# dask-contrib/dask-sql

Hardware: NVIDIA H100
Metric: rows/s on Q3-shaped filter->join->groupby (higher is better)
Workload: dtype f64

## Files before the change

dask-sql_b200/_lib.py:

```python
import ctypes as C
import os

HERE = os.path.dirname(os.path.abspath(__file__))
LIB_PATH = os.environ.get("B200SQL_LIB") or os.path.join(HERE, "libb200sql.so")

I64, F64, U8 = 0, 1, 2
U32 = 3
COL_SENTINEL = 1
MAX_COLS, MAX_TERMS, MAX_AGGS, MAX_KEYS, MAX_GATHER, MAX_PROG = 16, 8, 8, 4, 8, 64
TILE = 4096
EQ, NE, LT, LE, GT, GE, IS_NULL, IS_NOT_NULL, IS_TRUE = range(9)
AGG_SUM, AGG_SUMF, AGG_MIN, AGG_MAX, AGG_COUNT, AGG_AND, AGG_OR, AGG_XOR = range(8)
JOIN_INNER, JOIN_LEFT, JOIN_SEMI, JOIN_ANTI = range(4)
EMPTY_KEY = -(1 << 63)

OP_LOAD, OP_CONST_I, OP_CONST_F, OP_CONST_NULL, OP_I2F, OP_F2I = 0, 1, 2, 3, 4, 5
OP_ADD_I, OP_SUB_I, OP_MUL_I, OP_DIV_I, OP_NEG_I, OP_ABS_I, OP_MOD_I = 10, 11, 12, 13, 14, 15, 16
OP_ADD_F, OP_SUB_F, OP_MUL_F, OP_DIV_F, OP_NEG_F, OP_ABS_F, OP_SQRT_F = 20, 21, 22, 23, 24, 25, 26
OP_EQ_I, OP_EQ_F = 30, 40
OP_AND, OP_OR, OP_NOT, OP_ISNULL_I, OP_ISNULL_F, OP_CASE, OP_FILLNA, OP_ORD2F = 50, 51, 52, 53, 54, 55, 56, 57
OP_DATEPART, OP_ADDMONTHS = 60, 61
(DP_DAYS, DP_YEAR, DP_QUARTER, DP_MONTH, DP_DAY, DP_DOY, DP_DOW, DP_ISOWEEK, DP_HOUR, DP_MINUTE, DP_SECOND,
 DP_MILLISECOND, DP_MICROSECOND) = range(13)

# ... 48 lines not shown
                ("range", C.c_int64), ("table_keys", C.c_void_p), ("table_slots", C.c_void_p),
                ("cap", C.c_int64), ("dir", C.c_void_p)]


MAX_PEERS, PEER_MAX_ARRAYS = 16, 2 * MAX_AGGS + 1
PEER_SUM_F64, PEER_SUM_I64, PEER_MIN_I64, PEER_MAX_I64, PEER_AND_I64, PEER_OR_I64, PEER_XOR_I64 = range(7)
PEER_PRESENT_ROWS, PEER_PRESENT_INDICATOR, PEER_PRESENT_BITMAP = 1, 2, 3


class PeerMerge(C.Structure):
    _fields_ = [("world", C.c_int32), ("rank", C.c_int32), ("narrays", C.c_int32), ("presence_kind", C.c_int32),
                ("presence_array", C.c_int32), ("ops", C.c_int32 * PEER_MAX_ARRAYS),
                ("array_off", C.c_int64 * PEER_MAX_ARRAYS), ("bitmap_off", C.c_int64), ("signal_off", C.c_int64),
                ("peer_base", C.c_void_p * MAX_PEERS), ("out", C.c_void_p * PEER_MAX_ARRAYS),
                ("out_present", C.c_void_p), ("lo", C.c_int64), ("count", C.c_int64), ("local_ready", C.c_void_p),
                ("epoch", C.c_uint64)]


assert C.sizeof(Col) == 24 and C.sizeof(Term) == 32 and C.sizeof(Scan) == 656
assert C.sizeof(AggState) == 152 and C.sizeof(Instr) == 24 and C.sizeof(Prog) == 1544
assert C.sizeof(JoinTable) == 152 and C.sizeof(StarLookup) == 64 and C.sizeof(PeerMerge) == 544


def agg_identity(op):
    return {AGG_MIN: (1 << 63) - 1, AGG_MAX: -(1 << 63), AGG_AND: -1}.get(op, 0)


class B200SqlError(RuntimeError):
    pass


def _load():
    if not os.path.exists(LIB_PATH):
        raise ImportError(
            f"{LIB_PATH} is missing: the execution layer has no CPU fallback. Build it with "
            "`python __graft_entry__.py build` (nvcc -gencode arch=compute_90a,code=sm_90a).")
    return C.CDLL(LIB_PATH)


_lib = _load()
_lib.b2_last_error.restype = C.c_char_p
_lib.b2_num_tiles.restype = C.c_int64
_lib.b2_num_tiles.argtypes = [C.c_int64]
_lib.b2_stats_ws_bytes.restype = C.c_int64
_lib.b2_scan_agg_ws_bytes.restype = C.c_int64
_lib.b2_join_onepass_ws_bytes.restype = C.c_int64
_lib.b2_join_onepass_ws_bytes.argtypes = [C.c_int64]
_lib.b2_range_partition_ws_bytes.restype = C.c_int64
_lib.b2_range_partition_ws_bytes.argtypes = [C.c_int32]
_lib.b2_f64_to_ordered.restype = C.c_int64
_lib.b2_f64_to_ordered.argtypes = [C.c_double]
_lib.b2_ordered_to_f64.restype = C.c_double
_lib.b2_ordered_to_f64.argtypes = [C.c_int64]

_P = C.c_void_p
_SIGS = {
    "b2_version": [],
    "b2_device_info": [C.c_int32, C.POINTER(C.c_int32), C.POINTER(C.c_int64), C.POINTER(C.c_int32),
                       C.POINTER(C.c_int32), C.POINTER(C.c_int64)],
    "b2_d2h": [_P, _P, C.c_int64, _P],
    "b2_sync": [_P],
    "b2_memset": [_P, C.c_int32, C.c_int64, _P],
    "b2_col_stats": [C.POINTER(Col), C.c_int64, _P, _P, _P],
    "b2_expr_eval": [C.POINTER(Prog), C.POINTER(Col), C.c_int32, C.c_int64, _P, _P, _P],
    "b2_scan_agg": [C.POINTER(Scan), C.POINTER(Agg), C.c_int32, _P, _P, C.c_int32, _P, _P],
    "b2_select_count": [C.POINTER(Scan), _P, _P],
    "b2_select_write": [C.POINTER(Scan), _P, _P, C.c_int32, C.POINTER(C.c_int32), C.POINTER(_P),
                        C.POINTER(_P), _P],
    "b2_gather": [C.POINTER(Col), _P, C.c_int64, _P, _P, _P],
    "b2_groupby_dense": [C.POINTER(Scan), C.c_int32, C.c_int64, C.c_int64, C.POINTER(Agg), C.c_int32,
                         C.POINTER(AggState), _P],
    "b2_groupby_dense_grouped": [C.POINTER(Scan), C.c_int32, C.c_int64, C.c_int64, C.POINTER(Agg), C.c_int32,
                                 C.POINTER(AggState), _P],
    "b2_hot_slots": [C.POINTER(Col), C.c_int64, C.c_int64, C.c_int64, _P, _P],
    "b2_groupby_dense_hot": [C.POINTER(Scan), C.c_int32, C.c_int64, C.c_int64, C.POINTER(Agg), C.c_int32,
                             C.POINTER(AggState), _P, _P],
    "b2_groupby_dense_ordered": [C.POINTER(Scan), C.c_int32, C.c_int64, C.c_int64, C.POINTER(Agg), C.c_int32,
                                 C.POINTER(AggState), _P, _P],
    "b2_groupby_hash1": [C.POINTER(Scan), C.c_int32, _P, C.c_int64, C.POINTER(Agg), C.c_int32,
                         C.POINTER(AggState), _P, _P],
    "b2_groupby_hashk": [C.POINTER(Scan), C.POINTER(C.c_int32), C.c_int32, _P, _P, _P, C.c_int64,
                         C.POINTER(Agg), C.c_int32, C.POINTER(AggState), _P, _P],
    "b2_join_build": [C.POINTER(Col), C.c_int32, C.c_int64, _P, _P, C.c_int64, _P],
    "b2_join_build_dense": [C.POINTER(Col), C.c_int64, C.c_int64, C.c_int64, _P, _P, _P],
    "b2_join_count": [C.POINTER(Scan), C.POINTER(C.c_int32), C.POINTER(JoinTable), C.c_int32, _P, _P],
    "b2_join_write": [C.POINTER(Scan), C.POINTER(C.c_int32), C.POINTER(JoinTable), C.c_int32, _P, _P, _P,
                      _P, _P],
    "b2_join_write_gather": [C.POINTER(Scan), C.POINTER(C.c_int32), C.POINTER(JoinTable), C.c_int32, _P, _P, _P,
                             _P, C.c_int32, C.POINTER(C.c_int32), C.POINTER(_P), C.POINTER(_P), C.c_int32,
                             C.POINTER(Col), C.POINTER(_P), C.POINTER(_P), _P],
    "b2_join_key_layout": [C.POINTER(Col), C.c_int64, C.c_int64, C.c_int64, C.POINTER(Col), C.c_int32, C.c_int64,
                           _P, _P, _P, _P],
    "b2_join_write_gather_keyed": [C.POINTER(Scan), C.POINTER(C.c_int32), C.POINTER(JoinTable), C.c_int32, _P, _P,
                                   _P, _P, C.c_int32, C.POINTER(C.c_int32), C.POINTER(_P), C.POINTER(_P),
                                   C.c_int32, C.POINTER(Col), C.POINTER(C.c_int64), C.POINTER(_P), C.POINTER(_P),
                                   _P],
    "b2_join_onepass": [C.POINTER(Scan), C.POINTER(C.c_int32), C.POINTER(JoinTable), C.c_int32, C.c_int32, _P, C.c_int32,
                        C.POINTER(C.c_int32), C.POINTER(_P), C.POINTER(_P), C.c_int32, C.POINTER(Col),
                        C.POINTER(C.c_int64), C.POINTER(_P), C.POINTER(_P), _P],
    "b2_join_agg": [C.POINTER(Scan), C.c_int32, C.POINTER(JoinTable), C.c_int32, C.POINTER(Col), C.POINTER(C.c_int64),
                    C.POINTER(JoinAgg), C.c_int32, _P, _P, C.c_int32, _P, _P],
    "b2_range_partition_hist": [C.POINTER(Scan), C.c_int32, C.c_int64, C.c_int64, C.c_int32, C.c_int32, _P, _P],
    "b2_range_partition_scan": [C.c_int32, _P, _P],
    "b2_range_partition_scatter": [C.POINTER(Scan), C.c_int32, C.c_int64, C.c_int64, C.c_int32, C.c_int32, C.c_int32,
                                   C.POINTER(C.c_int32), _P, C.POINTER(_P), _P, _P],
    "b2_range_partition": [C.POINTER(Scan), C.c_int32, C.c_int64, C.c_int64, C.c_int32, C.c_int32, C.c_int32,
                           C.POINTER(C.c_int32), _P, C.POINTER(_P), _P, _P],
    "b2_iota": [_P, C.c_int64, _P],
    "b2_bitwise_combine": [_P, _P, C.c_int64, C.c_int32, _P],
    "b2_peer_merge": [C.POINTER(PeerMerge), _P],
    "b2_sort_by": [C.POINTER(Col), C.c_int64, C.c_int32, C.c_int32, _P, _P, _P],
    "b2_dense_slots": [C.POINTER(Col), C.c_int64, C.c_int64, C.c_int32, _P, _P],
    "b2_star_build_dense": [C.POINTER(Col), _P, C.c_int64, _P, C.c_int64, C.c_int64, _P, _P, _P],
    "b2_star_build_mark": [C.POINTER(Scan), C.c_int32, C.c_int64, C.c_int64, _P, _P, _P],
    "b2_star_build_rank": [_P, C.c_int64, _P],
    "b2_star_build_fill": [C.POINTER(Scan), C.c_int32, C.c_int32, C.c_int64, C.c_int64, C.c_int64, C.c_int32, _P,
                           _P, _P],
    "b2_star_build_fill_packed": [C.POINTER(Scan), C.c_int32, C.c_int32, C.c_int64, C.c_int64, C.c_int64,
                                  C.c_int32, _P, _P, C.c_int32, _P],
    "b2_star_build_hash": [C.POINTER(Col), _P, C.c_int64, _P, _P, _P, C.c_int64, _P, _P],
    "b2_star_agg": [C.POINTER(Scan), C.c_int32, C.POINTER(StarLookup), C.POINTER(Agg), C.c_int32,
                    C.POINTER(AggState), _P],
}

EXPORTS = sorted(list(_SIGS) + ["b2_last_error", "b2_num_tiles", "b2_stats_ws_bytes", "b2_scan_agg_ws_bytes",
                                "b2_sort_ws_bytes", "b2_join_onepass_ws_bytes", "b2_range_partition_ws_bytes",
                                "b2_f64_to_ordered", "b2_ordered_to_f64"])


call_times = {} if os.environ.get("B200SQL_CALL_TIMES") == "1" else None


def _wrap(name):
    fn = getattr(_lib, name)
    fn.restype = C.c_int32
    fn.argtypes = _SIGS[name]

    if call_times is not None:
        import time

        def call(*args):
            t0 = time.perf_counter()
            rc = fn(*args)
            rec = call_times.setdefault(name, [0, 0.0])
            rec[0] += 1
            rec[1] += time.perf_counter() - t0
            if rc != 0:
                raise B200SqlError(f"{name} failed ({rc}): {_lib.b2_last_error().decode()}")
            return rc

        call.__name__ = name
        return call

    def call(*args):
        rc = fn(*args)
        if rc != 0:
            raise B200SqlError(f"{name} failed ({rc}): {_lib.b2_last_error().decode()}")
        return rc

    call.__name__ = name
    return call


version = getattr(_lib, "b2_version")
version.restype = C.c_int32
device_info = _wrap("b2_device_info")
d2h = _wrap("b2_d2h")
sync = _wrap("b2_sync")
memset = _wrap("b2_memset")
col_stats = _wrap("b2_col_stats")
expr_eval = _wrap("b2_expr_eval")
scan_agg = _wrap("b2_scan_agg")
select_count = _wrap("b2_select_count")
select_write = _wrap("b2_select_write")
gather = _wrap("b2_gather")
groupby_dense = _wrap("b2_groupby_dense")
groupby_dense_ordered = _wrap("b2_groupby_dense_ordered")
groupby_dense_grouped = _wrap("b2_groupby_dense_grouped")
groupby_dense_hot = _wrap("b2_groupby_dense_hot")
hot_slots = _wrap("b2_hot_slots")
groupby_hash1 = _wrap("b2_groupby_hash1")
groupby_hashk = _wrap("b2_groupby_hashk")
join_build = _wrap("b2_join_build")
join_build_dense = _wrap("b2_join_build_dense")
join_count = _wrap("b2_join_count")
join_write = _wrap("b2_join_write")
join_write_gather = _wrap("b2_join_write_gather")
join_write_gather_keyed = _wrap("b2_join_write_gather_keyed")
join_key_layout = _wrap("b2_join_key_layout")
join_onepass = _wrap("b2_join_onepass")
join_onepass_ws_bytes = _lib.b2_join_onepass_ws_bytes
join_agg = _wrap("b2_join_agg")
range_partition = _wrap("b2_range_partition")
range_partition_hist = _wrap("b2_range_partition_hist")
range_partition_scan = _wrap("b2_range_partition_scan")
range_partition_scatter = _wrap("b2_range_partition_scatter")
range_partition_ws_bytes = _lib.b2_range_partition_ws_bytes
iota = _wrap("b2_iota")
bitwise_combine = _wrap("b2_bitwise_combine")
peer_merge = _wrap("b2_peer_merge")
sort_by = _wrap("b2_sort_by")
_lib.b2_sort_ws_bytes.restype = C.c_int64
_lib.b2_sort_ws_bytes.argtypes = [C.c_int64]
sort_ws_bytes = _lib.b2_sort_ws_bytes
dense_slots = _wrap("b2_dense_slots")
star_build_dense = _wrap("b2_star_build_dense")
star_build_mark = _wrap("b2_star_build_mark")
star_build_rank = _wrap("b2_star_build_rank")
star_build_fill = _wrap("b2_star_build_fill")
star_build_fill_packed = _wrap("b2_star_build_fill_packed")
star_build_hash = _wrap("b2_star_build_hash")
star_agg = _wrap("b2_star_agg")
num_tiles = _lib.b2_num_tiles
stats_ws_bytes = _lib.b2_stats_ws_bytes
scan_agg_ws_bytes = _lib.b2_scan_agg_ws_bytes
f64_to_ordered = _lib.b2_f64_to_ordered
ordered_to_f64 = _lib.b2_ordered_to_f64


def has_symbol(name):
    try:
        getattr(_lib, name)
        return True
    except AttributeError:
        return False
```

dask-sql_b200/csrc/groupby.cuh:

```cuda
#pragma once
#include "common.cuh"
#include "pipeline.cuh"
#include "warpagg.cuh"

#define B2_GB_R 8
#define B2_GB_ROWS_PER_BLOCK (B2_BLOCK * B2_GB_R)
#define B2_MAX_PROBE 1024

template <int R, class LD>
__device__ __forceinline__ void b2_dense_slots_of(const b2_scan_t& s, const LD& ld, int key_col, int64_t kmin,
                                                  int64_t nslots, int64_t (&slot)[R]) {
  const b2_col_t& kc = s.cols[key_col];
  bool full;
  const uint32_t bits = b2_eval_terms<R>(s, ld, full);
  int64_t key[R];
  ld.template load<R>(key_col, bits, full, key);
  uint32_t kvalid = bits;
  if (kc.valid) kvalid = b2_valid_bits<R>(kc.valid, ld.row0, bits);
#pragma unroll
  for (int j = 0; j < R; ++j) {
    slot[j] = -1;
    if ((bits >> j) & 1) {
      if (!((kvalid >> j) & 1)) slot[j] = nslots - 1;
      else {
// ... 210 lines not shown
b2_star_build_dense_kernel(const __grid_constant__ b2_col_t pk, const int32_t* __restrict__ sel, int64_t n_sel,
                           const int32_t* __restrict__ slot_of_row, int64_t kmin, int64_t range,
                           int32_t* __restrict__ lookup, int32_t* __restrict__ flags) {
  for (int64_t i = (int64_t)blockIdx.x * B2_BLOCK + threadIdx.x; i < n_sel; i += (int64_t)gridDim.x * B2_BLOCK) {
    const int64_t r = sel ? sel[i] : i;
    const int64_t raw = b2_load_raw(pk, r);
    if (b2_is_null(pk, r, raw)) continue;
    const uint64_t d = (uint64_t)raw - (uint64_t)kmin;
    if (d >= (uint64_t)range) continue;
    const int32_t old = atomicExch(lookup + d, slot_of_row[i]);
    if (old != -1) flags[0] = 1;
  }
}

__device__ __forceinline__ uint32_t b2_slot_word(uint32_t pos, int slot_bits) {
  return slot_bits == 16 ? pos >> 2 : __umulhi(pos, 0x55555556u);
}

template <bool FILL>
__global__ void __launch_bounds__(B2_BLOCK)
b2_star_build_scan_kernel(const __grid_constant__ b2_scan_t s, int pk_col, int grp_col, int64_t pk_min,
                          int64_t pk_range, int64_t grp_min, int32_t null_slot, uint64_t* __restrict__ dir,
                          void* __restrict__ slots, int slot_bits, int32_t* __restrict__ flags) {
  const int tile_off = (threadIdx.x >> 5) * (32 * B2_GB_R) + (threadIdx.x & 31);
  const b2_col_t& pc = s.cols[pk_col];
  const b2_col_t& gc = s.cols[grp_col];
  for (int64_t base = (int64_t)blockIdx.x * B2_GB_ROWS_PER_BLOCK; base < s.n;
       base += (int64_t)gridDim.x * B2_GB_ROWS_PER_BLOCK) {
    const b2_gld ld{&s, base + tile_off};
    bool full;
    const uint32_t bits = b2_eval_terms<B2_GB_R>(s, ld, full);
    int64_t pk[B2_GB_R];
    ld.template load<B2_GB_R>(pk_col, bits, full, pk);
    uint32_t live = bits;
    if (pc.valid) live &= b2_valid_bits<B2_GB_R>(pc.valid, ld.row0, bits);
#pragma unroll
    for (int j = 0; j < B2_GB_R; ++j) {
      const uint64_t d = (uint64_t)pk[j] - (uint64_t)pk_min;
      if (!(((live >> j) & 1) && d < (uint64_t)pk_range)) live &= ~(1u << j);
    }
    if (!FILL) {
#pragma unroll
      for (int j = 0; j < B2_GB_R; ++j) {
        if (!((live >> j) & 1)) continue;
        const uint64_t d = (uint64_t)pk[j] - (uint64_t)pk_min;
        const uint32_t b = 1u << (d & 31);
        if (atomicOr(reinterpret_cast<uint32_t*>(dir + (d >> 5)), b) & b) flags[0] = 1;
      }
    } else {
      int64_t grp[B2_GB_R];
      ld.template load<B2_GB_R>(grp_col, live, false, grp);
      uint32_t gnull = 0;
      if (gc.valid) gnull = live & ~b2_valid_bits<B2_GB_R>(gc.valid, ld.row0, live);
#pragma unroll
      for (int j = 0; j < B2_GB_R; ++j) {
        if (!((live >> j) & 1)) continue;
        const uint64_t d = (uint64_t)pk[j] - (uint64_t)pk_min;
        const uint64_t w = dir[d >> 5];
        const uint32_t pos = (uint32_t)(w >> 32) + __popc((uint32_t)w & ((1u << (d & 31)) - 1));
        const int32_t v = (gnull >> j) & 1 ? null_slot : (int32_t)(grp[j] - grp_min);
        if (slot_bits == 32) {
          static_cast<int32_t*>(slots)[pos] = v;
        } else {
          const uint32_t q = b2_slot_word(pos, slot_bits);
          const uint32_t sh = (pos - q * (64 / slot_bits)) * slot_bits;
          unsigned long long* p = reinterpret_cast<unsigned long long*>(slots) + q;
          const unsigned long long m = ((1ull << slot_bits) - 1) << sh;
          const unsigned long long e = ((unsigned long long)(uint32_t)v << sh) & m;
          unsigned long long old = 0, seen;
          while ((seen = atomicCAS(p, old, (old & ~m) | e)) != old) old = seen;
        }
      }
    }
  }
}

struct b2_scan_io_dir {
  uint64_t* dir;
  __device__ int64_t get(int64_t i) const { return __popc((uint32_t)dir[i]); }
  __device__ void put(int64_t i, int64_t v) const { dir[i] = (uint64_t)(uint32_t)dir[i] | ((uint64_t)v << 32); }
};

__global__ void __launch_bounds__(B2_SCAN_THREADS) b2_star_build_rank_kernel(uint64_t* __restrict__ dir, int64_t nwords) {
  b2_block_exclusive_scan(b2_scan_io_dir{dir}, nwords);
}

__global__ void __launch_bounds__(B2_BLOCK)
b2_star_build_hash_kernel(const __grid_constant__ b2_col_t pk, const int32_t* __restrict__ sel, int64_t n_sel,
                          const int32_t* __restrict__ slot_of_row, int64_t* __restrict__ tk,
                          int32_t* __restrict__ ts, int64_t cap, int32_t* __restrict__ flags) {
  for (int64_t i = (int64_t)blockIdx.x * B2_BLOCK + threadIdx.x; i < n_sel; i += (int64_t)gridDim.x * B2_BLOCK) {
    const int64_t r = sel ? sel[i] : i;
    const int64_t key = b2_load_raw(pk, r);
    if (b2_is_null(pk, r, key)) continue;
    if (key == B2_EMPTY_KEY) { flags[1] = 1; continue; }
    uint64_t h = b2_mix64((uint64_t)key) & (uint64_t)(cap - 1);
    bool done = false;
    for (int probe = 0; probe < B2_MAX_PROBE && !done; ++probe) {
      const unsigned long long old = atomicCAS(reinterpret_cast<unsigned long long*>(tk + h),
                                               (unsigned long long)B2_EMPTY_KEY, (unsigned long long)key);
      if (old == (unsigned long long)B2_EMPTY_KEY) { ts[h] = slot_of_row[i]; done = true; }
      else if (old == (unsigned long long)key) { flags[0] = 1; done = true; }
      else h = (h + 1) & (uint64_t)(cap - 1);
    }
    if (!done) flags[1] = 1;
  }
}

__device__ __forceinline__ int32_t b2_star_lookup(const b2_starlookup_t& lk, int64_t key) {
  if (lk.dense) {
    const uint64_t d = (uint64_t)key - (uint64_t)lk.kmin;
    return d < (uint64_t)lk.range ? b2_ld_keep_i32(lk.lookup + d) : -1;
  }
  uint64_t h = b2_mix64((uint64_t)key) & (uint64_t)(lk.cap - 1);
  for (int probe = 0; probe < B2_MAX_PROBE; ++probe) {
    const int64_t cur = __ldg(reinterpret_cast<const long long*>(lk.table_keys) + h);
    if (cur == key) return b2_ld_keep_i32(lk.table_slots + h);
    if (cur == B2_EMPTY_KEY) return -1;
    h = (h + 1) & (uint64_t)(lk.cap - 1);
  }
  return -1;
}

#define B2_STAR_R 16
template <int R, class LD>
__device__ __forceinline__ void b2_star_body(const b2_scan_t& s, const LD& ld, int fk_col, const b2_starlookup_t& lk,
                                             const b2_aggs_arg& aggs, const b2_aggstate_t& st) {
  const b2_col_t& kc = s.cols[fk_col];
  bool full0;
  const uint32_t inb = b2_bounds_bits<R>(ld.row0, s.n, full0);
  int64_t key[R];
  ld.template load<R>(fk_col, inb, full0, key);
  bool full;
  const uint32_t bits = b2_eval_terms<R>(s, ld, full);
  uint32_t live = bits;
  if (kc.valid) live &= b2_valid_bits<R>(kc.valid, ld.row0, bits);
  const bool prefetch = aggs.n > 0 && aggs.a[0].col >= 0;
  int64_t pre[R];
  int32_t found[R];
  int64_t slot[R];
  if (lk.dense == 2) {
    const uint64_t range = (uint64_t)lk.range;
    uint64_t w[R];
#pragma unroll
    for (int j = 0; j < R; ++j) {
      const uint64_t d = (uint64_t)key[j] - (uint64_t)lk.kmin;
      w[j] = (((live >> j) & 1) && d < range) ? (uint64_t)b2_ld_keep_i64(reinterpret_cast<const int64_t*>(lk.dir) + (d >> 5)) : 0;
    }
    if (prefetch) ld.template load<R>(aggs.a[0].col, live, false, pre);
    const int sb = lk.slot_bits;
    if (sb == 32) {
#pragma unroll
      for (int j = 0; j < R; ++j) {
        const uint32_t b = (uint32_t)((uint64_t)key[j] - (uint64_t)lk.kmin) & 31;
        const uint32_t bits = (uint32_t)w[j];
        found[j] = (bits >> b) & 1 ? b2_ld_keep_i32(lk.lookup + (uint32_t)(w[j] >> 32) + __popc(bits & ((1u << b) - 1))) : -1;
      }
    } else {
      const int k = 64 / sb;
      const uint64_t* words = reinterpret_cast<const uint64_t*>(lk.lookup);
#pragma unroll
      for (int j = 0; j < R; ++j) {
        const uint32_t b = (uint32_t)((uint64_t)key[j] - (uint64_t)lk.kmin) & 31;
        const uint32_t bits = (uint32_t)w[j];
        found[j] = -1;
        slot[j] = 0;
        if ((bits >> b) & 1) {
          const uint32_t pos = (uint32_t)(w[j] >> 32) + __popc(bits & ((1u << b) - 1));
          const uint32_t q = b2_slot_word(pos, sb);
          found[j] = (int32_t)((pos - q * k) * sb);
          slot[j] = b2_ld_keep_i64(reinterpret_cast<const int64_t*>(words + q));
        }
      }
      const uint64_t mask = (1ull << sb) - 1;
#pragma unroll
      for (int j = 0; j < R; ++j)
        found[j] = found[j] < 0 ? -1 : (int32_t)(((uint64_t)slot[j] >> found[j]) & mask);
    }
  } else if (lk.dense) {
    const uint64_t range = (uint64_t)lk.range;
#pragma unroll
    for (int j = 0; j < R; ++j) {
      const uint64_t d = (uint64_t)key[j] - (uint64_t)lk.kmin;
      found[j] = (((live >> j) & 1) && d < range) ? b2_ld_keep_i32(lk.lookup + d) : -1;
    }
  } else {
#pragma unroll
    for (int j = 0; j < R; ++j) {
      found[j] = -1;
      if (((live >> j) & 1) && key[j] != B2_EMPTY_KEY) found[j] = b2_star_lookup(lk, key[j]);
    }
  }
  if (lk.dense != 2 && prefetch) ld.template load<R>(aggs.a[0].col, live, false, pre);
#pragma unroll
  for (int j = 0; j < R; ++j) slot[j] = found[j];
  b2_apply_aggs<R>(s, ld, aggs.a, aggs.n, st, slot, pre);
}

template <bool PIPE>
__global__ void __launch_bounds__(PIPE ? B2_PIPE_THREADS : B2_BLOCK)
b2_star_agg_kernel(const __grid_constant__ b2_scan_t s, const __grid_constant__ b2_pipe_t pp, int fk_col,
                   const __grid_constant__ b2_starlookup_t lk, const __grid_constant__ b2_aggs_arg aggs,
                   const __grid_constant__ b2_aggstate_t st) {
  if (PIPE) b2_tile_pipeline(s, pp, [&](const auto& ld) { b2_star_body<B2_PIPE_R>(s, ld, fk_col, lk, aggs, st); });
  else b2_tile_direct<B2_STAR_R>(s, [&](const auto& ld) { b2_star_body<B2_STAR_R>(s, ld, fk_col, lk, aggs, st); });
}

extern "C" {

static int32_t b2_check_state(const b2_aggs_arg& aa, const b2_aggstate_t* st) {
  B2_REQUIRE(st, "null aggstate");
  for (int a = 0; a < aa.n; ++a) {
    if (aa.a[a].col < 0) { B2_REQUIRE(st->rows, "COUNT(*) needs aggstate.rows"); continue; }
    if (aa.a[a].op == B2_AGG_COUNT) B2_REQUIRE(st->cnt[a], "COUNT needs a cnt array");
    else B2_REQUIRE(st->acc[a], "aggregate needs an acc array");
  }
  return B2_OK;
}
static inline bool b2_pow2(int64_t x) { return x > 0 && (x & (x - 1)) == 0; }

static int32_t b2_groupby_dense_impl(const b2_scan_t* scan, int32_t key_col, int64_t kmin, int64_t nslots,
                                     const b2_agg_t* aggs, int32_t naggs, const b2_aggstate_t* st,
                                     unsigned long long* ticket, void* stream) {
  int32_t rc = b2_check_scan(scan);
  if (rc) return rc;
  b2_aggs_arg aa;
  if ((rc = b2_check_aggs(scan, aggs, naggs, &aa))) return rc;
  if ((rc = b2_check_state(aa, st))) return rc;
  B2_REQUIRE(key_col >= 0 && key_col < scan->ncols, "key column out of range");
  B2_REQUIRE(scan->cols[key_col].dtype == B2_I64 || scan->cols[key_col].dtype == B2_U8, "dense keys must be integers");
  B2_REQUIRE(nslots >= 2, "nslots must cover the key range plus the NULL slot");
  if (scan->n == 0) return B2_OK;
  b2_pipe_t pp;
  b2_make_pipe(*scan, &pp);
  if (ticket) pp.enabled = 0;
  if (pp.enabled) {
    int grid = b2_pipe_grid(b2_groupby_dense_kernel<true>, pp, scan->n);
    b2_groupby_dense_kernel<true><<<grid, B2_PIPE_THREADS, pp.smem_bytes, (cudaStream_t)stream>>>(*scan, pp, key_col, kmin, nslots, aa, *st, nullptr);
  } else {
    int64_t nblk = (scan->n + B2_GB_ROWS_PER_BLOCK - 1) / B2_GB_ROWS_PER_BLOCK;
    int grid = b2_wave_grid(b2_groupby_dense_kernel<false>, B2_BLOCK, nblk);
    b2_groupby_dense_kernel<false><<<grid, B2_BLOCK, 0, (cudaStream_t)stream>>>(*scan, pp, key_col, kmin, nslots, aa, *st, ticket);
  }
  B2_CHECK_LAUNCH("b2_groupby_dense_kernel");
  return B2_OK;
}

int32_t b2_groupby_dense(const b2_scan_t* scan, int32_t key_col, int64_t kmin, int64_t nslots,
                         const b2_agg_t* aggs, int32_t naggs, const b2_aggstate_t* st, void* stream) {
  return b2_groupby_dense_impl(scan, key_col, kmin, nslots, aggs, naggs, st, nullptr, stream);
}

int32_t b2_groupby_dense_grouped(const b2_scan_t* scan, int32_t key_col, int64_t kmin, int64_t nslots,
                                 const b2_agg_t* aggs, int32_t naggs, const b2_aggstate_t* st, void* stream) {
  int32_t rc = b2_check_scan(scan);
  if (rc) return rc;
  b2_aggs_arg aa;
  if ((rc = b2_check_aggs(scan, aggs, naggs, &aa))) return rc;
// ... 134 lines not shown
                       void* stream) {
  B2_REQUIRE(key && out_slot, "null argument");
  if (n <= 0) return B2_OK;
  int grid = b2_wave_grid(b2_dense_slots_kernel, B2_BLOCK, (n + B2_BLOCK - 1) / B2_BLOCK);
  b2_dense_slots_kernel<<<grid, B2_BLOCK, 0, (cudaStream_t)stream>>>(*key, n, kmin, null_slot, out_slot);
  B2_CHECK_LAUNCH("b2_dense_slots_kernel");
  return B2_OK;
}

int32_t b2_star_build_dense(const b2_col_t* pk, const int32_t* sel, int64_t n_sel, const int32_t* slot_of_row,
                            int64_t kmin, int64_t range, int32_t* lookup, int32_t* d_flags, void* stream) {
  B2_REQUIRE(pk && slot_of_row && lookup && d_flags, "null argument");
  B2_REQUIRE(pk->dtype == B2_I64, "dense lookup needs an int64 key");
  if (n_sel <= 0) return B2_OK;
  int grid = b2_wave_grid(b2_star_build_dense_kernel, B2_BLOCK, (n_sel + B2_BLOCK - 1) / B2_BLOCK);
  b2_star_build_dense_kernel<<<grid, B2_BLOCK, 0, (cudaStream_t)stream>>>(*pk, sel, n_sel, slot_of_row, kmin,
                                                                           range, lookup, d_flags);
  B2_CHECK_LAUNCH("b2_star_build_dense_kernel");
  return B2_OK;
}

static int32_t b2_star_build_pass(bool fill, const b2_scan_t* scan, int32_t pk_col, int32_t grp_col,
                                  int64_t pk_min, int64_t pk_range, int64_t grp_min, int32_t null_slot,
                                  uint64_t* dir, void* slots, int32_t slot_bits, int32_t* d_flags, void* stream) {
  int32_t rc = b2_check_scan(scan);
  if (rc) return rc;
  B2_REQUIRE(pk_col >= 0 && pk_col < scan->ncols && grp_col >= 0 && grp_col < scan->ncols, "column out of range");
  B2_REQUIRE(scan->cols[pk_col].dtype == B2_I64 && scan->cols[grp_col].dtype == B2_I64, "dense keys must be int64");
  B2_REQUIRE(pk_range > 0 && pk_range < ((int64_t)1 << 31), "bad range");
  if (scan->n == 0) return B2_OK;
  int64_t nblk = (scan->n + B2_GB_ROWS_PER_BLOCK - 1) / B2_GB_ROWS_PER_BLOCK;
  if (fill) {
    int grid = b2_wave_grid(b2_star_build_scan_kernel<true>, B2_BLOCK, nblk);
    b2_star_build_scan_kernel<true><<<grid, B2_BLOCK, 0, (cudaStream_t)stream>>>(*scan, pk_col, grp_col, pk_min, pk_range,
                                                                                  grp_min, null_slot, dir, slots, slot_bits, d_flags);
  } else {
    int grid = b2_wave_grid(b2_star_build_scan_kernel<false>, B2_BLOCK, nblk);
    b2_star_build_scan_kernel<false><<<grid, B2_BLOCK, 0, (cudaStream_t)stream>>>(*scan, pk_col, grp_col, pk_min, pk_range,
                                                                                   grp_min, null_slot, dir, slots, slot_bits, d_flags);
  }
  B2_CHECK_LAUNCH("b2_star_build_scan_kernel");
  return B2_OK;
}

int32_t b2_star_build_mark(const b2_scan_t* scan, int32_t pk_col, int64_t pk_min, int64_t pk_range, uint64_t* dir,
                           int32_t* d_flags, void* stream) {
  B2_REQUIRE(dir && d_flags, "null argument");
  return b2_star_build_pass(false, scan, pk_col, pk_col, pk_min, pk_range, 0, 0, dir, nullptr, 32, d_flags, stream);
}

int32_t b2_star_build_rank(uint64_t* dir, int64_t pk_range, void* stream) {
  B2_REQUIRE(dir, "null argument");
  B2_REQUIRE(pk_range > 0 && pk_range < ((int64_t)1 << 31), "bad range");
  b2_star_build_rank_kernel<<<1, B2_SCAN_THREADS, 0, (cudaStream_t)stream>>>(dir, (pk_range + 31) / 32);
  B2_CHECK_LAUNCH("b2_star_build_rank_kernel");
  return B2_OK;
}

int32_t b2_star_build_fill(const b2_scan_t* scan, int32_t pk_col, int32_t grp_col, int64_t pk_min,
                           int64_t pk_range, int64_t grp_min, int32_t null_slot, const uint64_t* dir,
                           int32_t* slots, void* stream) {
  return b2_star_build_fill_packed(scan, pk_col, grp_col, pk_min, pk_range, grp_min, null_slot, dir,
                                   reinterpret_cast<uint64_t*>(slots), 32, stream);
}

int32_t b2_star_build_fill_packed(const b2_scan_t* scan, int32_t pk_col, int32_t grp_col, int64_t pk_min,
                                  int64_t pk_range, int64_t grp_min, int32_t null_slot, const uint64_t* dir,
                                  uint64_t* slots, int32_t slot_bits, void* stream) {
  B2_REQUIRE(dir && slots, "null argument");
  B2_REQUIRE(slot_bits == 16 || slot_bits == 21 || slot_bits == 32, "slot_bits must be 16, 21 or 32");
  B2_REQUIRE(slot_bits == 32 || (null_slot >= 0 && null_slot < (1 << slot_bits)), "null_slot does not fit slot_bits");
  B2_REQUIRE(slot_bits == 32 || ((uintptr_t)slots & 7) == 0, "packed slots must be 8-byte aligned");
  return b2_star_build_pass(true, scan, pk_col, grp_col, pk_min, pk_range, grp_min, null_slot,
                            const_cast<uint64_t*>(dir), slots, slot_bits, nullptr, stream);
}

int32_t b2_star_build_hash(const b2_col_t* pk, const int32_t* sel, int64_t n_sel, const int32_t* slot_of_row,
                           int64_t* table_keys, int32_t* table_slots, int64_t cap, int32_t* d_flags,
                           void* stream) {
  B2_REQUIRE(pk && slot_of_row && table_keys && table_slots && d_flags, "null argument");
  B2_REQUIRE(pk->dtype == B2_I64, "star lookup needs an int64 key");
  B2_REQUIRE(b2_pow2(cap), "cap must be a power of two");
  if (n_sel <= 0) return B2_OK;
  int grid = b2_wave_grid(b2_star_build_hash_kernel, B2_BLOCK, (n_sel + B2_BLOCK - 1) / B2_BLOCK);
  b2_star_build_hash_kernel<<<grid, B2_BLOCK, 0, (cudaStream_t)stream>>>(*pk, sel, n_sel, slot_of_row, table_keys,
                                                                          table_slots, cap, d_flags);
  B2_CHECK_LAUNCH("b2_star_build_hash_kernel");
  return B2_OK;
}

int32_t b2_star_agg(const b2_scan_t* scan, int32_t fk_col, const b2_starlookup_t* lk, const b2_agg_t* aggs,
                    int32_t naggs, const b2_aggstate_t* st, void* stream) {
  int32_t rc = b2_check_scan(scan);
  if (rc) return rc;
  b2_aggs_arg aa;
  if ((rc = b2_check_aggs(scan, aggs, naggs, &aa))) return rc;
  if ((rc = b2_check_state(aa, st))) return rc;
  B2_REQUIRE(lk, "null lookup");
  B2_REQUIRE(fk_col >= 0 && fk_col < scan->ncols, "fk column out of range");
  B2_REQUIRE(scan->cols[fk_col].dtype == B2_I64, "fk must be int64");
  B2_REQUIRE(lk->dense >= 0 && lk->dense <= 2, "bad lookup kind");
  b2_starlookup_t l = *lk;
  if (l.dense == 2) {
    B2_REQUIRE(l.dir && l.lookup && l.range > 0 && l.range < ((int64_t)1 << 31), "bad bitmap lookup");
    if (l.slot_bits == 0) l.slot_bits = 32;
    B2_REQUIRE(l.slot_bits == 16 || l.slot_bits == 21 || l.slot_bits == 32, "slot_bits must be 0, 16, 21 or 32");
    B2_REQUIRE(l.slot_bits == 32 || ((uintptr_t)l.lookup & 7) == 0, "packed slots must be 8-byte aligned");
  }
  else if (l.dense) B2_REQUIRE(l.lookup && l.range > 0, "bad dense lookup");
  else B2_REQUIRE(l.table_keys && l.table_slots && b2_pow2(l.cap), "bad hash lookup");
  if (scan->n == 0) return B2_OK;
  b2_pipe_t pp;
  b2_make_pipe(*scan, &pp);
  if (pp.enabled) {
    int grid = b2_pipe_grid(b2_star_agg_kernel<true>, pp, scan->n);
    b2_star_agg_kernel<true><<<grid, B2_PIPE_THREADS, pp.smem_bytes, (cudaStream_t)stream>>>(*scan, pp, fk_col, l, aa, *st);
  } else {
    int64_t nblk = (scan->n + (int64_t)B2_BLOCK * B2_STAR_R - 1) / ((int64_t)B2_BLOCK * B2_STAR_R);
    int grid = b2_wave_grid(b2_star_agg_kernel<false>, B2_BLOCK, nblk);
    b2_star_agg_kernel<false><<<grid, B2_BLOCK, 0, (cudaStream_t)stream>>>(*scan, pp, fk_col, l, aa, *st);
  }
  B2_CHECK_LAUNCH("b2_star_agg_kernel");
  return B2_OK;
}

}
```

include/b200sql.h:

```cpp
#ifndef B200SQL_H
#define B200SQL_H
#include <stdint.h>
#ifdef __cplusplus
extern "C" {
#endif

#define B2_OK            0
#define B2_ERR_CUDA     -1
#define B2_ERR_ARG      -2

#define B2_I64 0
#define B2_F64 1
#define B2_U8  2
#define B2_U32 3

#define B2_MAX_COLS   16
#define B2_MAX_TERMS   8
#define B2_MAX_AGGS    8
#define B2_MAX_KEYS    4
#define B2_MAX_GATHER  8
#define B2_MAX_PROG   64
#define B2_TILE     4096

#define B2_EQ 0
// ... 273 lines not shown

int32_t b2_groupby_dense_ordered(const b2_scan_t* scan, int32_t key_col, int64_t kmin, int64_t nslots,
                                 const b2_agg_t* aggs, int32_t naggs, const b2_aggstate_t* st, uint64_t* d_ticket,
                                 void* stream);
int64_t b2_range_partition_ws_bytes(int32_t nbuckets);
int32_t b2_range_partition_hist(const b2_scan_t* scan, int32_t key_col, int64_t kmin, int64_t nslots, int32_t shift,
                                int32_t nbuckets, void* d_ws, void* stream);
int32_t b2_range_partition_scan(int32_t nbuckets, void* d_ws, void* stream);
int32_t b2_range_partition_scatter(const b2_scan_t* scan, int32_t key_col, int64_t kmin, int64_t nslots, int32_t shift,
                                   int32_t nbuckets, int32_t ncarry, const int32_t* carry_cols, int64_t* out_key,
                                   void* const* out_cols, void* d_ws, void* stream);
int32_t b2_range_partition(const b2_scan_t* scan, int32_t key_col, int64_t kmin, int64_t nslots, int32_t shift,
                           int32_t nbuckets, int32_t ncarry, const int32_t* carry_cols, int64_t* out_key,
                           void* const* out_cols, void* d_ws, void* stream);

int64_t b2_sort_ws_bytes(int64_t n);
int32_t b2_iota(int32_t* out, int64_t n, void* stream);
int32_t b2_sort_by(const b2_col_t* col, int64_t n, int32_t descending, int32_t nulls_first, int32_t* idx,
                   void* ws, void* stream);

int32_t b2_dense_slots(const b2_col_t* key, int64_t n, int64_t kmin, int32_t null_slot,
                       int32_t* out_slot, void* stream);

int32_t b2_star_build_dense(const b2_col_t* pk, const int32_t* sel, int64_t n_sel,
                            const int32_t* slot_of_row, int64_t kmin, int64_t range,
                            int32_t* lookup, int32_t* d_flags, void* stream);
int32_t b2_star_build_mark(const b2_scan_t* scan, int32_t pk_col, int64_t pk_min, int64_t pk_range,
                           uint64_t* dir, int32_t* d_flags, void* stream);
int32_t b2_star_build_rank(uint64_t* dir, int64_t pk_range, void* stream);
int32_t b2_star_build_fill(const b2_scan_t* scan, int32_t pk_col, int32_t grp_col, int64_t pk_min,
                           int64_t pk_range, int64_t grp_min, int32_t null_slot, const uint64_t* dir,
                           int32_t* slots, void* stream);
int32_t b2_star_build_fill_packed(const b2_scan_t* scan, int32_t pk_col, int32_t grp_col, int64_t pk_min,
                                  int64_t pk_range, int64_t grp_min, int32_t null_slot, const uint64_t* dir,
                                  uint64_t* slots, int32_t slot_bits, void* stream);
int32_t b2_star_build_hash(const b2_col_t* pk, const int32_t* sel, int64_t n_sel,
                           const int32_t* slot_of_row, int64_t* table_keys, int32_t* table_slots,
                           int64_t cap, int32_t* d_flags, void* stream);

typedef struct b2_starlookup {
  int32_t dense;
  int32_t slot_bits;
  const int32_t* lookup;
  int64_t kmin;
  int64_t range;
  const int64_t* table_keys;
  const int32_t* table_slots;
  int64_t cap;
  const uint64_t* dir;
} b2_starlookup_t;

int32_t b2_star_agg(const b2_scan_t* scan, int32_t fk_col, const b2_starlookup_t* lk,
                    const b2_agg_t* aggs, int32_t naggs, const b2_aggstate_t* st, void* stream);

#ifdef __cplusplus
}
#endif
#endif
```

Measured before the change: 77.79 billion.

## Shard star-join bitmap directory across cluster DSMEM and split work with side stream

Adds a thread-block-cluster variant of the star aggregation kernel. Each CTA in a 16-CTA cluster loads a slice of the bitmap directory into shared memory, and lookups go through distributed shared memory (mapa + ld.shared::cluster) instead of L2/global. SMs left outside the clusters run a non-DSMEM variant on a side stream over a share of the tiles, joined back with events. This aims to cut L2 traffic for random directory probes, at the cost of non-portable cluster sizes, cluster barriers and a more complex launch that only applies when the pipeline path is off and the lookup is a bitmap.

```diff
diff --git a/dask-sql_b200/_lib.py b/dask-sql_b200/_lib.py
--- a/dask-sql_b200/_lib.py
+++ b/dask-sql_b200/_lib.py
@@ -124,6 +124,8 @@
 _lib.b2_f64_to_ordered.argtypes = [C.c_double]
 _lib.b2_ordered_to_f64.restype = C.c_double
 _lib.b2_ordered_to_f64.argtypes = [C.c_int64]
+_lib.b2_star_dsmem_keys.restype = C.c_int64
+_lib.b2_star_dsmem_keys.argtypes = []
 
 _P = C.c_void_p
 _SIGS = {
@@ -197,7 +199,7 @@
 
 EXPORTS = sorted(list(_SIGS) + ["b2_last_error", "b2_num_tiles", "b2_stats_ws_bytes", "b2_scan_agg_ws_bytes",
                                 "b2_sort_ws_bytes", "b2_join_onepass_ws_bytes", "b2_range_partition_ws_bytes",
-                                "b2_f64_to_ordered", "b2_ordered_to_f64"])
+                                "b2_f64_to_ordered", "b2_ordered_to_f64", "b2_star_dsmem_keys"])
 
 
 call_times = {} if os.environ.get("B200SQL_CALL_TIMES") == "1" else None
@@ -283,6 +285,7 @@
 star_build_fill_packed = _wrap("b2_star_build_fill_packed")
 star_build_hash = _wrap("b2_star_build_hash")
 star_agg = _wrap("b2_star_agg")
+star_dsmem_keys = _lib.b2_star_dsmem_keys
 num_tiles = _lib.b2_num_tiles
 stats_ws_bytes = _lib.b2_stats_ws_bytes
 scan_agg_ws_bytes = _lib.b2_scan_agg_ws_bytes
diff --git a/dask-sql_b200/csrc/groupby.cuh b/dask-sql_b200/csrc/groupby.cuh
--- a/dask-sql_b200/csrc/groupby.cuh
+++ b/dask-sql_b200/csrc/groupby.cuh
@@ -357,9 +357,28 @@
 }
 
 #define B2_STAR_R 16
-template <int R, class LD>
+
+struct b2_dir_l2 {
+  const uint64_t* dir;
+  __device__ __forceinline__ uint64_t operator()(uint64_t d) const {
+    return (uint64_t)b2_ld_keep_i64(reinterpret_cast<const int64_t*>(dir) + (d >> 5));
+  }
+};
+struct b2_dir_dsmem {
+  uint32_t base, per, recip, shift;
+  __device__ __forceinline__ uint64_t operator()(uint64_t d) const {
+    const uint32_t w = (uint32_t)(d >> 5), owner = __umulhi(w, recip) >> shift;
+    uint32_t addr;
+    uint64_t v;
+    asm("mapa.shared::cluster.u32 %0, %1, %2;" : "=r"(addr) : "r"(base + (w - owner * per) * 8), "r"(owner));
+    asm volatile("ld.shared::cluster.u64 %0, [%1];" : "=l"(v) : "r"(addr));
+    return v;
+  }
+};
+
+template <int R, class LD, class DIR>
 __device__ __forceinline__ void b2_star_body(const b2_scan_t& s, const LD& ld, int fk_col, const b2_starlookup_t& lk,
-                                             const b2_aggs_arg& aggs, const b2_aggstate_t& st) {
+                                             const DIR& dir, const b2_aggs_arg& aggs, const b2_aggstate_t& st) {
   const b2_col_t& kc = s.cols[fk_col];
   bool full0;
   const uint32_t inb = b2_bounds_bits<R>(ld.row0, s.n, full0);
@@ -379,7 +398,7 @@
 #pragma unroll
     for (int j = 0; j < R; ++j) {
       const uint64_t d = (uint64_t)key[j] - (uint64_t)lk.kmin;
-      w[j] = (((live >> j) & 1) && d < range) ? (uint64_t)b2_ld_keep_i64(reinterpret_cast<const int64_t*>(lk.dir) + (d >> 5)) : 0;
+      w[j] = (((live >> j) & 1) && d < range) ? dir(d) : 0;
     }
     if (prefetch) ld.template load<R>(aggs.a[0].col, live, false, pre);
     const int sb = lk.slot_bits;
@@ -436,8 +455,45 @@
 b2_star_agg_kernel(const __grid_constant__ b2_scan_t s, const __grid_constant__ b2_pipe_t pp, int fk_col,
                    const __grid_constant__ b2_starlookup_t lk, const __grid_constant__ b2_aggs_arg aggs,
                    const __grid_constant__ b2_aggstate_t st) {
-  if (PIPE) b2_tile_pipeline(s, pp, [&](const auto& ld) { b2_star_body<B2_PIPE_R>(s, ld, fk_col, lk, aggs, st); });
-  else b2_tile_direct<B2_STAR_R>(s, [&](const auto& ld) { b2_star_body<B2_STAR_R>(s, ld, fk_col, lk, aggs, st); });
+  const b2_dir_l2 dir{lk.dir};
+  if (PIPE) b2_tile_pipeline(s, pp, [&](const auto& ld) { b2_star_body<B2_PIPE_R>(s, ld, fk_col, lk, dir, aggs, st); });
+  else b2_tile_direct<B2_STAR_R>(s, [&](const auto& ld) { b2_star_body<B2_STAR_R>(s, ld, fk_col, lk, dir, aggs, st); });
+}
+
+#define B2_STAR_CLUSTER 16
+#define B2_STAR_CLUSTER_BLOCK 512
+#define B2_STAR_CLUSTER_TILE ((int64_t)B2_STAR_CLUSTER_BLOCK * B2_STAR_R)
+__device__ __forceinline__ void b2_cluster_sync() {
+  asm volatile("barrier.cluster.arrive.release.aligned;\n\tbarrier.cluster.wait.acquire.aligned;" ::: "memory");
+}
+
+template <bool DSMEM>
+__global__ void __launch_bounds__(B2_STAR_CLUSTER_BLOCK, 1)
+b2_star_agg_cluster_kernel(const __grid_constant__ b2_scan_t s, int fk_col, const __grid_constant__ b2_starlookup_t lk,
+                           uint32_t per, uint32_t recip, uint32_t shift, int64_t t0, int64_t t1,
+                           const __grid_constant__ b2_aggs_arg aggs, const __grid_constant__ b2_aggstate_t st) {
+  const int tile_off = (threadIdx.x >> 5) * (32 * B2_STAR_R) + (threadIdx.x & 31);
+  auto tiles = [&](const auto& dir) {
+    for (int64_t t = t0 + blockIdx.x; t < t1; t += gridDim.x) {
+      const b2_gld ld{&s, t * B2_STAR_CLUSTER_TILE + tile_off};
+      b2_star_body<B2_STAR_R>(s, ld, fk_col, lk, dir, aggs, st);
+    }
+  };
+  if (!DSMEM) {
+    tiles(b2_dir_l2{lk.dir});
+    return;
+  }
+  extern __shared__ __align__(128) uint8_t b2_smem[];
+  uint64_t* slice = reinterpret_cast<uint64_t*>(b2_smem);
+  uint32_t me;
+  asm volatile("mov.u32 %0, %%cluster_ctarank;" : "=r"(me));
+  const uint32_t nwords = (uint32_t)((lk.range + 31) >> 5), w0 = me * per;
+  const uint32_t mine = w0 < nwords ? min(per, nwords - w0) : 0;
+  for (uint32_t i = threadIdx.x; i < mine; i += B2_STAR_CLUSTER_BLOCK)
+    slice[i] = (uint64_t)b2_ld_stream(reinterpret_cast<const int64_t*>(lk.dir) + w0 + i);
+  b2_cluster_sync();
+  tiles(b2_dir_dsmem{(uint32_t)__cvta_generic_to_shared(slice), per, recip, shift});
+  b2_cluster_sync();
 }
 
 extern "C" {
@@ -715,6 +771,84 @@
   return B2_OK;
 }
 
+static int64_t b2_star_dsmem_max_per() {
+  const char* e = getenv("B200SQL_STAR_DSMEM");
+  if (e && e[0] == '0') return 0;
+  int dev = 0, optin = 0;
+  if (cudaGetDevice(&dev) != cudaSuccess ||
+      cudaDeviceGetAttribute(&optin, cudaDevAttrMaxSharedMemoryPerBlockOptin, dev) != cudaSuccess) {
+    cudaGetLastError();
+    return 0;
+  }
+  return optin / 8;
+}
+
+static bool b2_star_dsmem_shape(int64_t nwords, uint32_t* per, uint32_t* recip, uint32_t* shift) {
+  int64_t p = (nwords + B2_STAR_CLUSTER - 1) / B2_STAR_CLUSTER;
+  if (p < 2) p = 2;
+  if (p > b2_star_dsmem_max_per()) return false;
+  uint32_t sh = 0;
+  while (((int64_t)2 << sh) < p) ++sh;
+  *per = (uint32_t)p;
+  *shift = sh;
+  *recip = (uint32_t)((((uint64_t)1 << (32 + sh)) + (uint64_t)p - 1) / (uint64_t)p);
+  return true;
+}
+
+static int b2_star_dsmem_clusters(size_t smem) {
+  static int last_dev = -1, last_clusters = 0;
+  static size_t last_smem = 0;
+  int dev = 0;
+  if (cudaGetDevice(&dev) != cudaSuccess) { cudaGetLastError(); return 0; }
+  if (dev == last_dev && smem == last_smem) return last_clusters;
+  int n = 0;
+  cudaLaunchConfig_t cfg = {};
+  cudaLaunchAttribute at[1];
+  at[0].id = cudaLaunchAttributeClusterDimension;
+  at[0].val.clusterDim.x = B2_STAR_CLUSTER;
+  at[0].val.clusterDim.y = 1;
+  at[0].val.clusterDim.z = 1;
+  cfg.gridDim = dim3(B2_STAR_CLUSTER);
+  cfg.blockDim = dim3(B2_STAR_CLUSTER_BLOCK);
+  cfg.dynamicSmemBytes = smem;
+  cfg.attrs = at;
+  cfg.numAttrs = 1;
+  if (cudaFuncSetAttribute(b2_star_agg_cluster_kernel<true>, cudaFuncAttributeNonPortableClusterSizeAllowed, 1) != cudaSuccess ||
+      cudaFuncSetAttribute(b2_star_agg_cluster_kernel<true>, cudaFuncAttributeMaxDynamicSharedMemorySize, (int)smem) != cudaSuccess ||
+      cudaOccupancyMaxActiveClusters(&n, b2_star_agg_cluster_kernel<true>, &cfg) != cudaSuccess) {
+    cudaGetLastError();
+    n = 0;
+  }
+  last_dev = dev;
+  last_smem = smem;
+  last_clusters = n;
+  return n;
+}
+
+static cudaError_t b2_star_side_stream(cudaStream_t* side, cudaEvent_t* fork, cudaEvent_t* join) {
+  static cudaStream_t streams[64];
+  static cudaEvent_t forks[64], joins[64];
+  int dev = 0;
+  cudaError_t e = cudaGetDevice(&dev);
+  if (e != cudaSuccess) return e;
+  if (dev < 0 || dev >= 64) return cudaErrorInvalidDevice;
+  if (!streams[dev]) {
+    if ((e = cudaEventCreateWithFlags(&forks[dev], cudaEventDisableTiming)) != cudaSuccess) return e;
+    if ((e = cudaEventCreateWithFlags(&joins[dev], cudaEventDisableTiming)) != cudaSuccess) return e;
+    if ((e = cudaStreamCreateWithFlags(&streams[dev], cudaStreamNonBlocking)) != cudaSuccess) return e;
+  }
+  *side = streams[dev];
+  *fork = forks[dev];
+  *join = joins[dev];
+  return cudaSuccess;
+}
+
+int64_t b2_star_dsmem_keys(void) {
+  const int64_t per = b2_star_dsmem_max_per();
+  if (per < 2 || b2_star_dsmem_clusters((size_t)per * 8) < 1) return 0;
+  return (int64_t)B2_STAR_CLUSTER * per * 32;
+}
+
 int32_t b2_star_agg(const b2_scan_t* scan, int32_t fk_col, const b2_starlookup_t* lk, const b2_agg_t* aggs,
                     int32_t naggs, const b2_aggstate_t* st, void* stream) {
   int32_t rc = b2_check_scan(scan);
@@ -738,7 +872,47 @@
   if (scan->n == 0) return B2_OK;
   b2_pipe_t pp;
   b2_make_pipe(*scan, &pp);
-  if (pp.enabled) {
+  uint32_t per, recip, shift;
+  int nclusters = 0;
+  if (!pp.enabled && l.dense == 2 && b2_star_dsmem_shape((l.range + 31) / 32, &per, &recip, &shift))
+    nclusters = b2_star_dsmem_clusters((size_t)per * 8);
+  if (nclusters > 0) {
+    const int64_t ntiles = (scan->n + B2_STAR_CLUSTER_TILE - 1) / B2_STAR_CLUSTER_TILE;
+    const int64_t free_sms = (int64_t)b2_sm_count() - (int64_t)nclusters * B2_STAR_CLUSTER;
+    const int64_t t2 = free_sms > 0 ? ntiles * free_sms * 9 / (free_sms * 9 + (int64_t)nclusters * B2_STAR_CLUSTER * 10) : 0;
+    const int64_t t1 = ntiles - t2;
+    const int64_t need = (t1 + B2_STAR_CLUSTER - 1) / B2_STAR_CLUSTER;
+    if (need < nclusters) nclusters = (int)need;
+    cudaStream_t mstream = (cudaStream_t)stream, side = nullptr;
+    cudaEvent_t fork = nullptr, join = nullptr;
+    if (t2 > 0) {
+      B2_CUDA_TRY(b2_star_side_stream(&side, &fork, &join));
+      B2_CUDA_TRY(cudaEventRecord(fork, mstream));
+      B2_CUDA_TRY(cudaStreamWaitEvent(side, fork, 0));
+    }
+    cudaLaunchConfig_t cfg = {};
+    cudaLaunchAttribute at[1];
+    at[0].id = cudaLaunchAttributeClusterDimension;
+    at[0].val.clusterDim.x = B2_STAR_CLUSTER;
+    at[0].val.clusterDim.y = 1;
+    at[0].val.clusterDim.z = 1;
+    cfg.gridDim = dim3(nclusters * B2_STAR_CLUSTER);
+    cfg.blockDim = dim3(B2_STAR_CLUSTER_BLOCK);
+    cfg.dynamicSmemBytes = (size_t)per * 8;
+    cfg.stream = mstream;
+    cfg.attrs = at;
+    cfg.numAttrs = 1;
+    B2_CUDA_TRY(cudaLaunchKernelEx(&cfg, b2_star_agg_cluster_kernel<true>, *scan, (int)fk_col, l, per, recip, shift,
+                                   (int64_t)0, t1, aa, *st));
+    if (t2 > 0) {
+      const int grid = (int)(free_sms < t2 ? free_sms : t2);
+      b2_star_agg_cluster_kernel<false><<<grid, B2_STAR_CLUSTER_BLOCK, 0, side>>>(*scan, fk_col, l, per, recip, shift,
+                                                                                   t1, ntiles, aa, *st);
+      B2_CHECK_LAUNCH("b2_star_agg_kernel");
+      B2_CUDA_TRY(cudaEventRecord(join, side));
+      B2_CUDA_TRY(cudaStreamWaitEvent(mstream, join, 0));
+    }
+  } else if (pp.enabled) {
     int grid = b2_pipe_grid(b2_star_agg_kernel<true>, pp, scan->n);
     b2_star_agg_kernel<true><<<grid, B2_PIPE_THREADS, pp.smem_bytes, (cudaStream_t)stream>>>(*scan, pp, fk_col, l, aa, *st);
   } else {
diff --git a/include/b200sql.h b/include/b200sql.h
--- a/include/b200sql.h
+++ b/include/b200sql.h
@@ -349,6 +349,7 @@
 
 int32_t b2_star_agg(const b2_scan_t* scan, int32_t fk_col, const b2_starlookup_t* lk,
                     const b2_agg_t* aggs, int32_t naggs, const b2_aggstate_t* st, void* stream);
+int64_t b2_star_dsmem_keys(void);
 
 #ifdef __cplusplus
 }
```

After: 81.72 billion, median of 6. 5.1% higher.

## Parallelize star-build rank scan across tiles and batch packed slot CAS writes

Applied to the files above, without the earlier changes.

Replaces the single-block exclusive scan over the directory words with a three-kernel tiled scan: per-tile popcount reduction, a single-block scan over the tile totals, then a per-tile write of ranks. This removes the serial single-block bottleneck when the key range is large. The fill pass now computes all positions first, writes 16-bit slots with plain stores instead of CAS loops, and issues the 21-bit CAS retries for all rows in a batch so they can be in flight together. It adds two extra kernel launches, and it relies on slot words not being shared across threads for the 16-bit direct stores.

```diff
diff --git a/dask-sql_b200/csrc/groupby.cuh b/dask-sql_b200/csrc/groupby.cuh
--- a/dask-sql_b200/csrc/groupby.cuh
+++ b/dask-sql_b200/csrc/groupby.cuh
@@ -286,37 +286,108 @@
       ld.template load<B2_GB_R>(grp_col, live, false, grp);
       uint32_t gnull = 0;
       if (gc.valid) gnull = live & ~b2_valid_bits<B2_GB_R>(gc.valid, ld.row0, live);
+      uint32_t pos[B2_GB_R];
+      int32_t v[B2_GB_R];
 #pragma unroll
       for (int j = 0; j < B2_GB_R; ++j) {
+        pos[j] = 0;
+        v[j] = 0;
         if (!((live >> j) & 1)) continue;
         const uint64_t d = (uint64_t)pk[j] - (uint64_t)pk_min;
         const uint64_t w = dir[d >> 5];
-        const uint32_t pos = (uint32_t)(w >> 32) + __popc((uint32_t)w & ((1u << (d & 31)) - 1));
-        const int32_t v = (gnull >> j) & 1 ? null_slot : (int32_t)(grp[j] - grp_min);
-        if (slot_bits == 32) {
-          static_cast<int32_t*>(slots)[pos] = v;
-        } else {
-          const uint32_t q = b2_slot_word(pos, slot_bits);
-          const uint32_t sh = (pos - q * (64 / slot_bits)) * slot_bits;
-          unsigned long long* p = reinterpret_cast<unsigned long long*>(slots) + q;
-          const unsigned long long m = ((1ull << slot_bits) - 1) << sh;
-          const unsigned long long e = ((unsigned long long)(uint32_t)v << sh) & m;
-          unsigned long long old = 0, seen;
-          while ((seen = atomicCAS(p, old, (old & ~m) | e)) != old) old = seen;
+        pos[j] = (uint32_t)(w >> 32) + __popc((uint32_t)w & ((1u << (d & 31)) - 1));
+        v[j] = (gnull >> j) & 1 ? null_slot : (int32_t)(grp[j] - grp_min);
+      }
+      if (slot_bits == 32 || slot_bits == 16) {
+#pragma unroll
+        for (int j = 0; j < B2_GB_R; ++j) {
+          if (!((live >> j) & 1)) continue;
+          if (slot_bits == 32) static_cast<int32_t*>(slots)[pos[j]] = v[j];
+          else static_cast<uint16_t*>(slots)[pos[j]] = (uint16_t)v[j];
+        }
+      } else {
+        unsigned long long e[B2_GB_R], old[B2_GB_R];
+        uint32_t q[B2_GB_R], sh[B2_GB_R];
+#pragma unroll
+        for (int j = 0; j < B2_GB_R; ++j) {
+          q[j] = b2_slot_word(pos[j], 21);
+          sh[j] = (pos[j] - q[j] * 3) * 21;
+          e[j] = ((unsigned long long)(uint32_t)v[j] & 0x1FFFFFull) << sh[j];
+          old[j] = 0;
+        }
+        unsigned long long* w = reinterpret_cast<unsigned long long*>(slots);
+        for (uint32_t pend = live; pend;) {
+          unsigned long long seen[B2_GB_R];
+#pragma unroll
+          for (int j = 0; j < B2_GB_R; ++j)
+            if ((pend >> j) & 1) seen[j] = atomicCAS(w + q[j], old[j], (old[j] & ~(0x1FFFFFull << sh[j])) | e[j]);
+#pragma unroll
+          for (int j = 0; j < B2_GB_R; ++j) {
+            if (!((pend >> j) & 1)) continue;
+            if (seen[j] == old[j]) pend &= ~(1u << j);
+            else old[j] = seen[j];
+          }
         }
       }
     }
   }
 }
 
-struct b2_scan_io_dir {
+#define B2_RANK_PER_THREAD 8
+#define B2_RANK_TILE (B2_BLOCK * B2_RANK_PER_THREAD)
+
+__device__ __forceinline__ uint32_t* b2_rank_half(uint64_t* dir, int64_t i) {
+  return reinterpret_cast<uint32_t*>(dir + i) + 1;
+}
+
+template <bool WRITE>
+__global__ void __launch_bounds__(B2_BLOCK) b2_star_rank_tile_kernel(uint64_t* __restrict__ dir, int64_t nwords) {
+  __shared__ int warp_sums[B2_WARPS];
+  __shared__ uint32_t tile_off;
+  const int lane = threadIdx.x & 31, warp = threadIdx.x >> 5;
+  const int64_t t0 = (int64_t)blockIdx.x * B2_RANK_TILE;
+  const int64_t i0 = t0 + (int64_t)threadIdx.x * B2_RANK_PER_THREAD;
+  if (WRITE && threadIdx.x == 0) tile_off = *b2_rank_half(dir, t0);
+  uint32_t bits[B2_RANK_PER_THREAD];
+  int tsum = 0;
+#pragma unroll
+  for (int k = 0; k < B2_RANK_PER_THREAD; ++k) {
+    bits[k] = i0 + k < nwords ? (uint32_t)dir[i0 + k] : 0u;
+    tsum += __popc(bits[k]);
+  }
+  int incl = tsum;
+#pragma unroll
+  for (int o = 1; o < 32; o <<= 1) {
+    const int t = __shfl_up_sync(FULL_MASK, incl, o);
+    if (lane >= o) incl += t;
+  }
+  if (lane == 31) warp_sums[warp] = incl;
+  __syncthreads();
+  if (!WRITE) {
+    if (threadIdx.x == 0) {
+      int total = 0;
+      for (int w = 0; w < B2_WARPS; ++w) total += warp_sums[w];
+      *b2_rank_half(dir, t0) = (uint32_t)total;
+    }
+    return;
+  }
+  uint32_t r = tile_off + (uint32_t)(incl - tsum);
+  for (int w = 0; w < warp; ++w) r += (uint32_t)warp_sums[w];
+#pragma unroll
+  for (int k = 0; k < B2_RANK_PER_THREAD; ++k) {
+    if (i0 + k < nwords) dir[i0 + k] = (uint64_t)bits[k] | ((uint64_t)r << 32);
+    r += __popc(bits[k]);
+  }
+}
+
+struct b2_scan_io_tile_off {
   uint64_t* dir;
-  __device__ int64_t get(int64_t i) const { return __popc((uint32_t)dir[i]); }
-  __device__ void put(int64_t i, int64_t v) const { dir[i] = (uint64_t)(uint32_t)dir[i] | ((uint64_t)v << 32); }
+  __device__ int64_t get(int64_t t) const { return *b2_rank_half(dir, t * B2_RANK_TILE); }
+  __device__ void put(int64_t t, int64_t v) const { *b2_rank_half(dir, t * B2_RANK_TILE) = (uint32_t)v; }
 };
 
-__global__ void __launch_bounds__(B2_SCAN_THREADS) b2_star_build_rank_kernel(uint64_t* __restrict__ dir, int64_t nwords) {
-  b2_block_exclusive_scan(b2_scan_io_dir{dir}, nwords);
+__global__ void __launch_bounds__(B2_SCAN_THREADS) b2_star_rank_carry_kernel(uint64_t* __restrict__ dir, int64_t ntiles) {
+  b2_block_exclusive_scan(b2_scan_io_tile_off{dir}, ntiles);
 }
 
 __global__ void __launch_bounds__(B2_BLOCK)
@@ -678,8 +749,14 @@
 int32_t b2_star_build_rank(uint64_t* dir, int64_t pk_range, void* stream) {
   B2_REQUIRE(dir, "null argument");
   B2_REQUIRE(pk_range > 0 && pk_range < ((int64_t)1 << 31), "bad range");
-  b2_star_build_rank_kernel<<<1, B2_SCAN_THREADS, 0, (cudaStream_t)stream>>>(dir, (pk_range + 31) / 32);
-  B2_CHECK_LAUNCH("b2_star_build_rank_kernel");
+  const int64_t nwords = (pk_range + 31) / 32;
+  const int64_t ntiles = (nwords + B2_RANK_TILE - 1) / B2_RANK_TILE;
+  b2_star_rank_tile_kernel<false><<<(unsigned)ntiles, B2_BLOCK, 0, (cudaStream_t)stream>>>(dir, nwords);
+  B2_CHECK_LAUNCH("b2_star_rank_tile_kernel<false>");
+  b2_star_rank_carry_kernel<<<1, B2_SCAN_THREADS, 0, (cudaStream_t)stream>>>(dir, ntiles);
+  B2_CHECK_LAUNCH("b2_star_rank_carry_kernel");
+  b2_star_rank_tile_kernel<true><<<(unsigned)ntiles, B2_BLOCK, 0, (cudaStream_t)stream>>>(dir, nwords);
+  B2_CHECK_LAUNCH("b2_star_rank_tile_kernel<true>");
   return B2_OK;
 }
 
```

After: 68.42 billion before, 70.98 billion after, median of 6. 1.04x the previous value.
